# gudovskiy/contextflow

Hardware: AMD Instinct MI355X
Metric: samples/s fwd+logdet (log p(x) (B,M)), CIFAR-10C conv flow (higher is better)
Workload: dtype f32

## Files before the change

contextflow_amd/csrc/cf_step.hip:

```cpp
#include "cf_step_common.h"
#include <cstdlib>

namespace {

struct StepArgs {
    const float* x;
    float* z;
    float* ldj;
    const float* ws;
    int B;
    int64_t xbs;
    bool sq;
    hipStream_t s;
    float* dbg = nullptr;
    const float* sb = nullptr;
    StepTape tp = kNoTape;
};

constexpr int kPrepBatch = 16;
struct StepPackBatch {
    const float *Wm[kPrepBatch], *t[kPrepBatch], *logs[kPrepBatch], *w1[kPrepBatch], *b1[kPrepBatch], *w2[kPrepBatch], *b2[kPrepBatch],
        *w3[kPrepBatch], *b3[kPrepBatch];
    float* ws[kPrepBatch];
    int pieces;
// ... 166 lines not shown
            }
        }
    }
}

template <class G, bool SQ, int CTX = 0, bool DUMP = false, bool DBG = false>
__global__ __launch_bounds__(256, G::MINW) void k_flow_step(const float* __restrict__ x, float* __restrict__ z,
                                                   float* __restrict__ ldj_acc, const float* __restrict__ ws, int B,
                                                   int64_t xbs, float* __restrict__ dbg_arg, int flags,
                                                   const float* __restrict__ sb, StepTape tp) {
    float* const dbg = DBG ? dbg_arg : nullptr;
    constexpr int C = G::C, HW = G::HW, W = G::W, H = G::H, PIX = G::PIX, HALF = G::HALF, HID = G::HID;
    constexpr int PTW = G::PTW, RT03 = G::RT03, RT1 = G::RT1;
    constexpr int WPX = 32 * PTW;
    constexpr int XI = C * PTW / 8;
    extern __shared__ __align__(16) float lds[];
    float* Y0 = lds;
    float* H1 = lds + HALF * PIX;

    const int tid = threadIdx.x, lane = tid & 63, wave = tid >> 6, li = lane & 31, lk = lane >> 5;
    const int ntiles = (B + G::SPW - 1) / G::SPW;
    const int64_t dbg_cols = (int64_t)ntiles * PIX;
    (void)flags;

    int pix[PTW], pin[PTW];
#pragma unroll
    for (int q = 0; q < PTW; ++q) {
        pix[q] = (wave * PTW + q) * 32 + li;
        pin[q] = pix[q] % HW;
    }

    float4 xr[XI];
    const int tile = blockIdx.x;
    x_load<G, SQ>(xr, x, xbs, tile, B, wave, lane);
    {
        const float* __restrict__ wsl = ws;
        const int b0 = tile * G::SPW;
        int smp[PTW];
        bool live[PTW];
#pragma unroll
        for (int q = 0; q < PTW; ++q) { smp[q] = b0 + pix[q] / HW; live[q] = smp[q] < B; }

        x_to_lds<G, SQ>(xr, H1, wave, lane);
        cf_wave_sync();

        f32x16 acc0[RT03][PTW];
#pragma unroll
        for (int rt = 0; rt < RT03; ++rt)
#pragma unroll
            for (int q = 0; q < PTW; ++q) acc0[rt][q] = bias_tile(wsl + G::OFF_B0 + rt * 32, lk);
        dense_phase<G, G::KS0, G::NG0, RT03>(acc0, ws_rsrc(wsl, G::WS_FLOATS), G::OFF_A0, H1, pix, lane);
        float y1[PTW][HALF <= 16 ? 8 : 16];
#pragma unroll
        for (int q = 0; q < PTW; ++q)
#pragma unroll
            for (int r = 0; r < (HALF <= 16 ? 8 : 16); ++r) {
                const int idx = tile_row(r, lk);
                if (idx < HALF) Y0[idx * PIX + pix[q]] = acc0[0][q][r];
                y1[q][r] = (HALF <= 16) ? acc0[0][q][r + 8] : acc0[RT03 - 1][q][r];
            }
        cf_wave_sync();
        z_store<G>(z, Y0, b0, 0, B, wave, lane);
        if constexpr (DUMP) rows_store_t<G, HALF, HALF>(tp.y0, Y0, b0, B, wave, lane);
        if (dbg) {
            __syncthreads();
            for (int e = tid; e < HALF * PIX; e += 256) dbg[(int64_t)(e / PIX) * dbg_cols + (int64_t)tile * PIX + (e % PIX)] = Y0[e];
            __syncthreads();
        }

        f32x16 acc3[RT03][PTW];
        if constexpr (CTX == 0) {
            conditioner_net<G, 0, DUMP>(acc3, lds, wsl, pix, pin, lane, tid, dbg, dbg_cols, tile, nullptr, nullptr, tp, B);
        } else {
            int soff[PTW];
#pragma unroll
            for (int q = 0; q < PTW; ++q) soff[q] = min(smp[q], B - 1) * (CTX == 1 ? C : HID);
            conditioner_net<G, CTX, DUMP>(acc3, lds, wsl, pix, pin, lane, tid, dbg, dbg_cols, tile, sb, soff, tp, B);
        }

        float lsum[PTW];
#pragma unroll
        for (int q = 0; q < PTW; ++q) {
            lsum[q] = 0.f;
#pragma unroll
            for (int r = 0; r < (HALF <= 16 ? 8 : 16); ++r) {
                const int idx = tile_row(r, lk);
                if (idx < HALF) {
                    const float tt = acc3[0][q][r];
                    const float raw = (HALF <= 16) ? acc3[0][q][r + 8] : acc3[RT03 - 1][q][r];
                    const float ls = cf_log_scale(raw);
                    Y0[idx * PIX + pix[q]] = fmaf(y1[q][r], __expf(ls), tt);
                    lsum[q] += ls;
                    if constexpr (DUMP) {
                        if (live[q]) {
                            const int64_t o = ((int64_t)smp[q] * HALF + idx) * HW + pin[q];
                            tp.ls[o] = ls;
                            tp.y1[o] = y1[q][r];
                        }
                    }
                    if (dbg) {
                        float* d = dbg + (int64_t)(C + 2 * HID) * dbg_cols + (int64_t)tile * PIX + pix[q];
                        d[(int64_t)idx * dbg_cols] = tt;
                        d[(int64_t)(HALF + idx) * dbg_cols] = raw;
                    }
                }
            }
        }
        cf_wave_sync();
        z_store<G>(z, Y0, b0, HALF, B, wave, lane);
        cf_wave_sync();

        constexpr int SEG = HW < 32 ? HW : 32;
        float v[PTW];
#pragma unroll
        for (int q = 0; q < PTW; ++q) {
            v[q] = lsum[q];
#pragma unroll
            for (int o = 1; o < SEG; o <<= 1) v[q] += __shfl_xor(v[q], o, 64);
            v[q] += __shfl_xor(v[q], 32, 64);
        }
        if constexpr (HW <= 32 * PTW) {
            constexpr int TPS = HW >= 32 ? HW / 32 : 1;
#pragma unroll
            for (int q = 0; q < PTW; q += TPS) {
                float sum = v[q];
#pragma unroll
                for (int i = 1; i < TPS; ++i) sum += v[q + i];
                if (lk == 0 && (li % SEG) == 0 && live[q]) ldj_acc[smp[q]] += wsl[0] + sum;
            }
        } else {
            constexpr int TPS = HW / 32;
#pragma unroll
            for (int q = 0; q < PTW; ++q)
                if (lane == 0) Y0[wave * WPX + q] = v[q];
            __syncthreads();
            if (tid < G::SPW && b0 + tid < B) {
                float sum = 0.f;
#pragma unroll
                for (int i = 0; i < TPS; ++i) {
                    const int t = tid * TPS + i;
                    sum += Y0[(t / PTW) * WPX + (t % PTW)];
                }
                ldj_acc[b0 + tid] += wsl[0] + sum;
            }
            __syncthreads();
        }
    }
}

typedef float f32x4 __attribute__((ext_vector_type(4)));

#ifndef CF_G16W_MINW
#define CF_G16W_MINW 4
#endif
#ifdef CF_ABL_NOCONF
#define CF_ROWIDX(r, lg) ((r) * PIX + ((lg) * 16 & 63))
#else
#define CF_ROWIDX(r, lg) (((r) + (lg)) * PIX)
#endif
template <class G, bool SQ, bool DBG = false, bool DUMP = false, int CTX = 0>
__device__ __forceinline__ void flow_step_small_body(const float* x, float* z, float* __restrict__ ldj_acc, const float* __restrict__ ws,
                                                     int B, int64_t xbs, float* __restrict__ dbg, StepTape tp,
                                                     const float* __restrict__ sb = nullptr) {
    static_assert(G::SMALL, "16x16 images, one sample per workgroup, C <= 16");
    static_assert(CTX == 0 || !G::HID16, "the per-sample bias is wired into the 32-row conditioner phases (C = 16)");
    constexpr int C = G::C, W = 16, H = 16, PIX = 256, HALF = G::HALF, HID = G::HID, PTW = G::PTW;
    constexpr int XI = C * PTW / 8;
    extern __shared__ __align__(16) float lds[];
    float* Y0 = lds;
    float* H1 = lds + HALF * PIX;
    const int tid = threadIdx.x, lane = tid & 63, wave = tid >> 6, l15 = lane & 15, lg = lane >> 4;
    const int tile = blockIdx.x;
    const int colb = wave * 64 + l15;

    float4 xr[XI];
    x_load<G, SQ>(xr, x, xbs, tile, B, wave, lane);
    const ws_rsrc_t rs = ws_rsrc(ws, G::WS_FLOATS);
    x_to_lds<G, SQ>(xr, H1, wave, lane);
    if constexpr (G::LDS_W > 0) {
        float* WL = lds + (HALF + HID) * PIX;
#pragma unroll
        for (int i = 0; i < G::LDS_W / 1024; ++i)
            *reinterpret_cast<float4*>(WL + (i * 256 + tid) * 4) = ws_frag(rs, tid, G::OFF_AW + i * 1024);
    }
    cf_wave_sync();

    f32x4 acc0[4];
    {
        const float4 b = *reinterpret_cast<const float4*>(ws + G::OFF_SB0 + 4 * lg);
#pragma unroll
        for (int ct = 0; ct < 4; ++ct) { acc0[ct][0] = b.x; acc0[ct][1] = b.y; acc0[ct][2] = b.z; acc0[ct][3] = b.w; }
#pragma unroll
        for (int g = 0; g < G::SG0; ++g) {
            const float4 a = ws_frag(rs, lane, G::OFF_SA0 + g * 256);
#pragma unroll
            for (int e = 0; e < 4; ++e)
                if (4 * (4 * g + e) < C) {
#pragma unroll
                    for (int ct = 0; ct < 4; ++ct)
                        acc0[ct] = __builtin_amdgcn_mfma_f32_16x16x4f32(f4e(a, e), H1[CF_ROWIDX(4 * (4 * g + e), lg) + colb + 16 * ct],
                                                                        acc0[ct], 0, 0, 0);
                }
        }
    }
#pragma unroll
    for (int ct = 0; ct < 4; ++ct)
#pragma unroll
        for (int j = 0; j < 2; ++j)
            if (2 * lg + j < HALF) Y0[(2 * lg + j) * PIX + colb + 16 * ct] = acc0[ct][j];
    cf_wave_sync();
    z_store<G>(z, Y0, tile, 0, B, wave, lane);
    if constexpr (DUMP) rows_store_t<G, HALF, HALF>(tp.y0, Y0, tile, B, wave, lane);
    const int64_t dbg_cols = (int64_t)B * PIX;
    auto dump = [&](const float* plane, int rows, int row0) {
        __syncthreads();
        for (int e = tid; e < rows * PIX; e += 256) dbg[(int64_t)(row0 + e / PIX) * dbg_cols + (int64_t)tile * PIX + (e % PIX)] = plane[e];
        __syncthreads();
    };
    if constexpr (DBG) dump(Y0, HALF, 0);
    auto plane_mask_store = [&](unsigned* __restrict__ m) {
        const int li = lane & 31, lk = lane >> 5;
#pragma unroll
        for (int q = 0; q < PTW; ++q) {
            unsigned b = 0;
#pragma unroll
            for (int r = 0; r < 8; ++r) b |= (H1[tile_row(r, lk) * PIX + (wave * PTW + q) * 32 + li] > 0.f ? 1u : 0u) << r;
            m[((int64_t)tile * G::NPT + wave * PTW + q) * 64 + lane] = b;
        }
    };
    (void)plane_mask_store;

    if constexpr (G::DBF) {
        static_assert(!DUMP && !DBG && CTX != 2, "evaluation form only");
        direct_bf16_phases<G>(lds, ws, rs, lane, wave);
    } else if constexpr (!G::HID16) {
        const int li = lane & 31;
        int pix[PTW], pin[PTW];
#pragma unroll
        for (int q = 0; q < PTW; ++q) { pix[q] = (wave * PTW + q) * 32 + li; pin[q] = pix[q]; }
        f32x16 unused[G::RT03][PTW];
        int soff[PTW];
#pragma unroll
        for (int q = 0; q < PTW; ++q) soff[q] = tile * HID;
        conditioner_net<G, CTX == 2 ? 2 : 0, DUMP, 2>(unused, lds, ws, pix, pin, lane, tid, DBG ? dbg : nullptr, dbg_cols, tile,
// ... 43 lines not shown
#pragma unroll
            for (int d = 0; d < 3; ++d) {
                int xx = l15 + d - 1;
                xx = xx < 0 ? -xx : (xx >= W ? 2 * (W - 1) - xx : xx);
                xo[d] = HALF * PIX + lg * PIX + xx;
            }
#pragma unroll
            for (int tap = 0; tap < 9; ++tap) {
                const float4 a = ws_frag(rs, lane, G::OFF_SA2 + tap * 256);
#pragma unroll
                for (int ct = 0; ct < 4; ++ct) {
                    int yy = wave * 4 + ct + tap / 3 - 1;
                    yy = yy < 0 ? -yy : (yy >= H ? 2 * (H - 1) - yy : yy);
                    const int src = xo[tap % 3] + yy * W;
#pragma unroll
                    for (int e = 0; e < 4; ++e)
                        a2[ct] = __builtin_amdgcn_mfma_f32_16x16x4f32(f4e(a, e), lds[src + 4 * e * PIX], a2[ct], 0, 0, 0);
                }
            }
        }
        __syncthreads();
#pragma unroll
        for (int ct = 0; ct < 4; ++ct)
#pragma unroll
            for (int r = 0; r < 4; ++r) H1[(4 * lg + r) * PIX + colb + 16 * ct] = cf_relu(a2[ct][r]);
        if constexpr (DUMP) { rows_store_t<G, HID, HID>(tp.h2, H1, tile, B, wave, lane); plane_mask_store(tp.m2); }
        if constexpr (DBG) dump(H1, HID, C + HID);
        }
    }
    cf_wave_sync();

    f32x4 acc3[4];
    {
        const float4 b = *reinterpret_cast<const float4*>(ws + G::OFF_SB3 + 4 * lg);
#pragma unroll
        for (int ct = 0; ct < 4; ++ct) { acc3[ct][0] = b.x; acc3[ct][1] = b.y; acc3[ct][2] = b.z; acc3[ct][3] = b.w; }
#pragma unroll
        for (int g = 0; g < G::SG3; ++g) {
            const float4 a = ws_frag(rs, lane, G::OFF_SA3 + g * 256);
#pragma unroll
            for (int e = 0; e < 4; ++e)
                if (4 * (4 * g + e) < HID) {
#pragma unroll
                    for (int ct = 0; ct < 4; ++ct)
                        acc3[ct] = __builtin_amdgcn_mfma_f32_16x16x4f32(f4e(a, e), H1[CF_ROWIDX(4 * (4 * g + e), lg) + colb + 16 * ct],
                                                                        acc3[ct], 0, 0, 0);
                }
        }
    }
    if constexpr (CTX == 1) {
#pragma unroll
        for (int r = 0; r < 4; ++r) {
            const int ch = chan_of_row16<G>(4 * lg + r);
            const float add = ch >= 0 ? sb[(int64_t)tile * C + ch] : 0.f;
#pragma unroll
            for (int ct = 0; ct < 4; ++ct) acc3[ct][r] += add;
        }
    }
    float lsum = 0.f;
#pragma unroll
    for (int ct = 0; ct < 4; ++ct)
#pragma unroll
        for (int j = 0; j < 2; ++j)
            if (2 * lg + j < HALF) {
                const float ls = cf_log_scale(acc3[ct][j + 2]);
                Y0[(2 * lg + j) * PIX + colb + 16 * ct] = fmaf(acc0[ct][j + 2], __expf(ls), acc3[ct][j]);
                lsum += ls;
                if constexpr (DUMP) {
                    const int64_t o = ((int64_t)tile * HALF + 2 * lg + j) * PIX + colb + 16 * ct;
                    tp.ls[o] = ls;
                    tp.y1[o] = acc0[ct][j + 2];
                }
                if constexpr (DBG) {
                    float* d = dbg + (int64_t)(C + 2 * HID) * dbg_cols + (int64_t)tile * PIX + colb + 16 * ct;
                    d[(int64_t)(2 * lg + j) * dbg_cols] = acc3[ct][j];
                    d[(int64_t)(HALF + 2 * lg + j) * dbg_cols] = acc3[ct][j + 2];
                }
            }
    cf_wave_sync();
    z_store<G>(z, Y0, tile, HALF, B, wave, lane);
    cf_wave_sync();
    lsum = cf_wave_sum(lsum);
    if (lane == 0) Y0[wave * 64] = lsum;
    __syncthreads();
    if (tid == 0 && tile < B) ldj_acc[tile] += ws[0] + ((Y0[0] + Y0[64]) + (Y0[128] + Y0[192]));
}
#ifndef CF_G16WB_MINW
#define CF_G16WB_MINW 3
#endif
#ifndef CF_G16DB_MINW
#define CF_G16DB_MINW 3
#endif
template <class G, bool SQ, bool DBG = false, bool DUMP = false, int CTX = 0>
__global__ __launch_bounds__(256, G::DBF ? CF_G16DB_MINW : G::BF16S ? CF_G16WB_MINW : (G::WINO && DUMP) ? 3 : (G::WINO && G::C == 16) ? CF_G16W_MINW : G::MINW) void k_flow_step_small(const float* __restrict__ x, float* __restrict__ z,
                                                                  float* __restrict__ ldj_acc, const float* __restrict__ ws,
                                                                  int B, int64_t xbs, float* __restrict__ dbg, StepTape tp,
                                                                  const float* __restrict__ sb = nullptr) {
    flow_step_small_body<G, SQ, DBG, DUMP, CTX>(x, z, ldj_acc, ws, B, xbs, dbg, tp, sb);
}
constexpr int kChain = 4;
struct WsChain { const float* ws[kChain]; };
template <class G, bool SQ>
__global__ __launch_bounds__(256, (G::WINO && G::C == 16) ? CF_G16W_MINW : G::MINW) void k_flow_step_small_chain(const float* x, float* z, float* __restrict__ ldj_acc,
                                                                                   const WsChain wc, int nsteps, int B, int64_t xbs) {
    flow_step_small_body<G, SQ>(x, z, ldj_acc, wc.ws[0], B, xbs, nullptr, kNoTape);
    for (int st = 1; st < nsteps; ++st) {
        __syncthreads();
        flow_step_small_body<G, false>(z, z, ldj_acc, wc.ws[st], B, (int64_t)G::C * G::HW, nullptr, kNoTape);
    }
}
template <class G>
int launch_step_small_chain(const StepArgs& a, const WsChain& wc, int n) {
    const auto k = a.sq ? k_flow_step_small_chain<G, true> : k_flow_step_small_chain<G, false>;
    k<<<dim3(a.B), dim3(256), (size_t)G::LDS_FLOATS * sizeof(float), a.s>>>(a.x, a.z, a.ldj, wc, n, a.B, a.xbs);
    return 0;
}

template <class G, bool DBG = false, bool DUMP = false, int CTX = 0>
int launch_step_small(const StepArgs& a) {
    auto k = k_flow_step_small<G, false, DBG, DUMP, CTX>;
    if constexpr (CTX == 0) { if (a.sq) k = k_flow_step_small<G, true, DBG, DUMP, CTX>; }
    k<<<dim3(a.B), dim3(256), (size_t)G::LDS_FLOATS * sizeof(float), a.s>>>(a.x, a.z, a.ldj, a.ws, a.B, a.xbs, a.dbg, a.tp, a.sb);
    return 0;
}

#ifdef CF_RS_TICKS
#define RS_TICK_INIT long long tacc_[12]; for (int k_ = 0; k_ < 12; ++k_) tacc_[k_] = 0; long long tprev_ = __builtin_readcyclecounter();
#define RS_TICK(k) { const long long tn_ = __builtin_readcyclecounter(); tacc_[k] += tn_ - tprev_; tprev_ = tn_; }
#define RS_TICK_DUMP if (blockIdx.x == 0 && lane == 0) for (int k_ = 0; k_ < 12; ++k_) z[wave * 16 + k_] = (float)tacc_[k_];
#else
#define RS_TICK_INIT
#define RS_TICK(k)
#define RS_TICK_DUMP
#endif
template <class G, int NPT, bool SQ, bool DUMP = false, int KS = 2>
__device__ __forceinline__ void flow_step_rs_body(const float* x, float* z, float* __restrict__ ldj_acc, const float* __restrict__ ws, int B,
                                                  int64_t xbs, StepTape tp = kNoTape) {
    constexpr int C = G::C, HW = G::HW, W = G::W, H = G::H, HALF = G::HALF, HID = G::HID, HP = G::HP;
    constexpr int PIXR = 32 * NPT, SPWR = PIXR / HW, RT1 = G::RT1, RT03 = G::RT03;
    static_assert(RT1 * NPT == 4 && RT03 * NPT == 2 && HP == HALF && PIXR % HW == 0, "row-split geometry");
    __shared__ __align__(16) float lds[(2 * C + HID + 2 * C) * PIXR];
    float* XP = lds;
    float* Y = XP + C * PIXR;
    float* H1 = Y + C * PIXR;
    float* T = H1 + HID * PIXR;
    static_assert(KS == 2, "eight waves: the only form that is instantiated and tested");
    constexpr int NTH = 256 * KS;
    const int tid = threadIdx.x, lane = tid & 63, wave = tid >> 6, li = lane & 31, lk = lane >> 5;
    const int w4 = wave & 3, kh2 = wave >> 2;
    const int b0 = blockIdx.x * SPWR;
    const ws_rsrc_t rs = ws_rsrc(ws, G::WS_FLOATS);
    RS_TICK_INIT
// ... 411 lines not shown
        __syncthreads();
        flow_step_rs16_body<G, false>(z, z, ldj_acc, wc.ws[st], B, (int64_t)G::C * G::HW);
    }
}
template <class G>
int launch_step_rs16_chain(const StepArgs& a, const WsChain& wc, int n) {
    const auto k = a.sq ? k_flow_step_rs16_chain<G, true> : k_flow_step_rs16_chain<G, false>;
    k<<<dim3(a.B), dim3(256), 0, a.s>>>(a.x, a.z, a.ldj, wc, n, a.B, a.xbs);
    return 0;
}
template <class G, bool DUMP = false>
int launch_step_rs16(const StepArgs& a) {
    const auto k = a.sq ? k_flow_step_rs16<G, true, DUMP> : k_flow_step_rs16<G, false, DUMP>;
    k<<<dim3(a.B), dim3(256), 0, a.s>>>(a.x, a.z, a.ldj, a.ws, a.B, a.xbs, a.tp);
    return 0;
}

extern "C" int cf_slogdet_inverse_batch(int n, const float* const* Wm, int C, float* const* logabsdet, float* const* inv, cf_stream_t stream);

template <class G>
int launch_prepare(const StepPackBatch& pb, int n, float* const* winv, hipStream_t s) {
    float* lad[kPrepBatch];
    for (int i = 0; i < n; ++i) lad[i] = pb.ws[i] + 1;
    int rc = cf_slogdet_inverse_batch(n, pb.Wm, G::C, lad, winv, (cf_stream_t)s);
    if (rc) return rc;
    int blocks = (G::WS_FLOATS + 255) / 256;
    if (blocks > 512) blocks = 512;
    k_step_pack<G><<<dim3(blocks, n), dim3(256), 0, s>>>(pb);
    return 0;
}

template <class G, bool SQ, int CTX, bool DUMP, bool DBG>
int launch_step_sq(const StepArgs& a) {
    constexpr size_t lds_bytes = (size_t)G::LDS_FLOATS * sizeof(float);
    if (lds_bytes > 64 * 1024) {
        static std::atomic<uint64_t> raised{0};
        if (int rc_ = cf_raise_dynamic_lds((const void*)k_flow_step<G, SQ, CTX, DUMP, DBG>, 160 * 1024, raised, __func__)) return rc_;
    }
    const int grid = (a.B + G::SPW - 1) / G::SPW;
    k_flow_step<G, SQ, CTX, DUMP, DBG><<<dim3(grid), dim3(256), lds_bytes, a.s>>>(a.x, a.z, a.ldj, a.ws, a.B, a.xbs, a.dbg, 0, a.sb, a.tp);
    return 0;
}
template <class G, int CTX = 0, bool DUMP = false, bool DBG = false>
int launch_step(const StepArgs& a) {
    if constexpr (CTX == 0) { if (a.sq) return launch_step_sq<G, true, CTX, DUMP, DBG>(a); }
    return launch_step_sq<G, false, CTX, DUMP, DBG>(a);
}

template <class G> struct GeoInv {
    static constexpr int RTI = (G::C + 31) / 32;
    static constexpr int OFF_WINV = 0;
    static constexpr int OFF_BI = ((G::C * G::C + 3) / 4) * 4;
    static constexpr int OFF_AI = OFF_BI + RTI * 32;
    static constexpr int WS_FLOATS = OFF_AI + G::NG0 * RTI * 256;
};

template <class G>
__global__ __launch_bounds__(256) void k_step_pack_inv(const float* __restrict__ t, const float* __restrict__ logs,
                                                       float* __restrict__ wsi) {
    using I = GeoInv<G>;
    const int gtid = blockIdx.x * 256 + threadIdx.x, gsz = gridDim.x * 256;
    const float* Winv = wsi + I::OFF_WINV;
    for (int c = gtid; c < I::RTI * 32; c += gsz) {
        float s = 0.f;
        if (c < G::C)
            for (int k = 0; k < G::C; ++k) s = fmaf(Winv[c * G::C + k], t[k], s);
// ... 559 lines not shown
```

contextflow_amd/csrc/cf_step_common.h:

```cpp
#pragma once
#include <type_traits>
#include "cf_common.h"
#include <math.h>

namespace {


typedef float f32x16 __attribute__((ext_vector_type(16)));

constexpr int kWaves = 4;

template <int C_, int H_, int W_, int SPW_, int PIPE_ = 1, int ABL_ = 0, int PATCH_ = 0>
struct Geo {
    static constexpr int C = C_, H = H_, W = W_, SPW = SPW_, PIPE = PIPE_, ABL = ABL_, PATCH = PATCH_;
    static constexpr int HW = H * W;
    static constexpr int PIX = SPW * HW;
    static constexpr int HALF = C / 2;
    static constexpr int HID = 2 * C;
    static constexpr int NPT = PIX / 32;
    static constexpr int PTW = NPT / kWaves;
    static constexpr int HP = HALF <= 16 ? 16 : 32;
    static constexpr int R03 = 2 * HP;
    static constexpr int RT03 = R03 / 32;
    static constexpr int RT1 = (HID + 31) / 32;
// ... 42 lines not shown
    static constexpr int LDS_W = (CF_WINO_LDSW && PIPE_ == 3 && HID == 16 && H == 16 && W == 16 && SPW == 1) ? 16 * HID * HID : 0;
    static constexpr int DBF_FLOATS = 3 * PIX * HID / 2;
    static constexpr int LDS_FLOATS = (DBF && DBF_FLOATS > (HALF + HID) * RS) ? DBF_FLOATS : (HALF + HID) * RS + LDS_W;
    static constexpr int MINW = (160 * 1024) / (LDS_FLOATS * 4) >= 4 ? 4 : ((160 * 1024) / (LDS_FLOATS * 4) >= 2 ? 2 : 1);
    static_assert(PIX % 128 == 0 && PTW >= 1, "workgroup must own a multiple of 128 pixels");
    static_assert(!W24 || (H == 4 && W == 4 && SPW == 8) || (H == 8 && W == 8 && SPW == 4),
                  "F(2x4, 3x3): 4x4 images, 8 samples = one column tile of 16 output tiles; 8x8 images, 4 samples = two column tiles");
    static_assert(HID % 8 == 0 && C % 4 == 0, "channel counts must fill whole k-steps");
    static_assert((HW & (HW - 1)) == 0 && (W & (W - 1)) == 0, "power-of-two images");
};

template <class G> __host__ __device__ constexpr int chan_of_row(int p) {
    return ((p % G::HP) < G::HALF) ? (p / G::HP) * G::HALF + (p % G::HP) : -1;
}

template <class G> __host__ __device__ constexpr int chan_of_row16(int p) {
    return (2 * (p >> 2) + (p & 1) < G::HALF) ? ((p & 2) ? G::HALF : 0) + 2 * (p >> 2) + (p & 1) : -1;
}

__device__ __forceinline__ f32x16 bias_tile(const float* __restrict__ bias32, int lk) {
    f32x16 a;
#pragma unroll
    for (int q = 0; q < 4; ++q) {
        const float4 v = *reinterpret_cast<const float4*>(bias32 + 8 * q + 4 * lk);
        a[4 * q + 0] = v.x; a[4 * q + 1] = v.y; a[4 * q + 2] = v.z; a[4 * q + 3] = v.w;
    }
    return a;
}
__device__ __forceinline__ int tile_row(int r, int lk) { return (r & 3) + 8 * (r >> 2) + 4 * lk; }
__device__ __forceinline__ float cf_relu(float x) { return __int_as_float(max(__float_as_int(x), 0)); }
__device__ __forceinline__ float cf_log_scale(float raw) { return fmaf(-4.0f, __builtin_amdgcn_rcpf(__expf(raw) + 1.0f), 2.0f); }
__device__ __forceinline__ float f4e(const float4& v, int e) { return e == 0 ? v.x : e == 1 ? v.y : e == 2 ? v.z : v.w; }

template <int RT, int PTW>
struct GroupOps {
    float4 a[RT];
    float b[4][PTW];
};

template <int RT, int PTW>
__device__ __forceinline__ void group_mma(f32x16 (&acc)[RT][PTW], const GroupOps<RT, PTW>& o, int nsteps) {
#pragma unroll
    for (int e = 0; e < 4; ++e) {
        if (e < nsteps) {
#pragma unroll
            for (int q = 0; q < PTW; ++q)
#pragma unroll
                for (int rt = 0; rt < RT; ++rt)
                    acc[rt][q] = __builtin_amdgcn_mfma_f32_32x32x2f32(f4e(o.a[rt], e), o.b[e][q], acc[rt][q], 0, 0, 0);
        }
    }
}

typedef __amdgpu_buffer_rsrc_t ws_rsrc_t;
__device__ __forceinline__ ws_rsrc_t ws_rsrc(const float* ws, int floats) {
    return __builtin_amdgcn_make_buffer_rsrc(const_cast<float*>(ws), 0, floats * 4, 0x00020000);
}
__device__ __forceinline__ float4 ws_frag(ws_rsrc_t rs, int lane, int foff) {
    typedef int i32x4_t __attribute__((ext_vector_type(4)));
    const i32x4_t v = __builtin_amdgcn_raw_buffer_load_b128(rs, lane * 16, foff * 4, 0);
    return make_float4(__int_as_float(v.x), __int_as_float(v.y), __int_as_float(v.z), __int_as_float(v.w));
}

template <class G, int KS, int NG, int RT, class FRAG>
__device__ __forceinline__ void dense_phase_impl(f32x16 (&acc)[RT][G::PTW], FRAG frag,
                                                 const float* __restrict__ plane, const int (&pix)[G::PTW], int lane) {
    const int lk = lane >> 5;
    cf_wave_sync();
    GroupOps<RT, G::PTW> ops[2];
    auto load = [&](int g, GroupOps<RT, G::PTW>& o) {
#pragma unroll
        for (int rt = 0; rt < RT; ++rt) o.a[rt] = frag(g * RT + rt);
#pragma unroll
        for (int e = 0; e < 4; ++e)
#pragma unroll
            for (int q = 0; q < G::PTW; ++q)
                o.b[e][q] = (4 * g + e < KS) ? plane[(2 * (4 * g + e) + lk) * G::RS + pix[q]] : 0.f;
    };
    load(0, ops[0]);
#pragma unroll
    for (int g = 0; g < NG; ++g) {
        if (g + 1 < NG) load(g + 1, ops[(g + 1) & 1]);
        __builtin_amdgcn_sched_barrier(0);
        group_mma<RT, G::PTW>(acc, ops[g & 1], KS - 4 * g);
    }
}
template <class G, int KS, int NG, int RT>
__device__ __forceinline__ void dense_phase(f32x16 (&acc)[RT][G::PTW], const float4* __restrict__ frags,
                                            const float* __restrict__ plane, const int (&pix)[G::PTW], int lane) {
    dense_phase_impl<G, KS, NG, RT>(acc, [&](int i) { return frags[i * 64 + lane]; }, plane, pix, lane);
}
template <class G, int KS, int NG, int RT>
__device__ __forceinline__ void dense_phase(f32x16 (&acc)[RT][G::PTW], ws_rsrc_t rs, int foff,
// ... 99 lines not shown
    const uint64_t p = reinterpret_cast<uint64_t>(base);
    return cf_i32x4{(int)(uint32_t)p, (int)((uint32_t)(p >> 32) & 0xffffu), bytes, 0x00020000};
}
__device__ __forceinline__ void tile_store_b128(const cf_i32x4 rs, int voff, int soff, const float4 v) {
    typedef float f32x4s __attribute__((ext_vector_type(4)));
    const f32x4s d = {v.x, v.y, v.z, v.w};
#if CF_STREAM_NT
    asm volatile("buffer_store_dwordx4 %0, %1, %2, %3 offen nt\n\ts_nop 1" : : "v"(d), "v"(voff), "s"(rs), "s"(soff) : "memory");
#else
    asm volatile("buffer_store_dwordx4 %0, %1, %2, %3 offen\n\ts_nop 1" : : "v"(d), "v"(voff), "s"(rs), "s"(soff) : "memory");
#endif
}

template <class G, int NROWS, int CT>
__device__ __forceinline__ void rows_store_t(float* __restrict__ dst, const float* __restrict__ plane, int tb0, int B,
                                             int wave, int lane) {
    constexpr int WPX = 32 * G::PTW, HW = G::HW, PIX = G::RS, RPI = 256 / WPX;
    const cf_i32x4 rs = tile_rsrc_words(dst + (int64_t)tb0 * CT * HW, min(B - tb0, G::SPW) * CT * HW * 4);
    const int idx0 = lane / (WPX / 4), col = wave * WPX + 4 * (lane % (WPX / 4));
    const int voff = ((col / HW) * CT * HW + idx0 * HW + col % HW) * 4;
    cf_wave_sync();
#ifdef CF_ABL_NOSTORE
    if (tb0 >= 0) return;
#endif
#pragma unroll
    for (int i = 0; i < (NROWS + RPI - 1) / RPI; ++i) {
        if (NROWS % RPI == 0 || idx0 + i * RPI < NROWS) {
            const float4 v = *reinterpret_cast<const float4*>(&plane[(idx0 + i * RPI) * PIX + col]);
            tile_store_b128(rs, voff, i * RPI * HW * 4, v);
        }
    }
    cf_wave_sync();
}
template <class G>
__device__ __forceinline__ void rows_store_unsq(float* __restrict__ dst, const float* __restrict__ plane, int tb0, int B,
                                                int wave, int lane) {
    constexpr int WPX = 32 * G::PTW, HW = G::HW, W = G::W, PIX = G::RS, C = G::C, Q4 = WPX / 4;
    static_assert(C % 4 == 0 && W % 4 == 0, "channel quadruples, 4 pixels of one image row");
    cf_wave_sync();
    for (int it = lane; it < (C / 2) * Q4; it += 64) {
        const int j = it / Q4, col = wave * WPX + 4 * (it - j * Q4);
        const int smp = tb0 + col / HW, p = col % HW, yy = p / W, xx = p - yy * W;
        if (smp < B) {
            const float4 a = *reinterpret_cast<const float4*>(&plane[(2 * j) * PIX + col]);
            const float4 b = *reinterpret_cast<const float4*>(&plane[(2 * j + 1) * PIX + col]);
            float* d = dst + (int64_t)smp * C * HW + (j >> 1) * 4 * HW + (2 * yy + (j & 1)) * 2 * W + 2 * xx;
            *reinterpret_cast<float4*>(d) = make_float4(a.x, b.x, a.y, b.y);
            *reinterpret_cast<float4*>(d + 4) = make_float4(a.z, b.z, a.w, b.w);
        }
    }
    cf_wave_sync();
}
template <class G, int NROWS, int CT>
__device__ __forceinline__ void rows_load_t(const float* __restrict__ src, float* __restrict__ plane, int tb0, int B,
                                            int wave, int lane) {
    typedef int i32x4_t __attribute__((ext_vector_type(4)));
    constexpr int WPX = 32 * G::PTW, HW = G::HW, PIX = G::RS, RPI = 256 / WPX;
    const ws_rsrc_t rs = tile_rsrc<G, CT>(src, tb0, B);
    const int idx0 = lane / (WPX / 4), col = wave * WPX + 4 * (lane % (WPX / 4));
    const int voff = ((col / HW) * CT * HW + idx0 * HW + col % HW) * 4;
    cf_wave_sync();
#pragma unroll
    for (int i = 0; i < (NROWS + RPI - 1) / RPI; ++i) {
        if (NROWS % RPI == 0 || idx0 + i * RPI < NROWS) {
            const i32x4_t v = __builtin_amdgcn_raw_buffer_load_b128(rs, voff, i * RPI * HW * 4, 0);
            *reinterpret_cast<float4*>(&plane[(idx0 + i * RPI) * PIX + col]) =
// ... 53 lines not shown
__device__ __forceinline__ void winograd_phase2(float* __restrict__ lds, const float* __restrict__ wsl, ws_rsrc_t rs, int lane,
                                                     int wave) {
    constexpr int W = G::W, H = G::H, HW = G::HW, PIX = G::PIX, HALF = G::HALF, HID = G::HID, RT16 = G::RT16, KG4 = G::KG4;
    constexpr int RSPLIT = G::PTW == 1 ? 2 : 1, NT = G::PTW * RSPLIT / 2, NCW = 4 / RSPLIT, RTW = RT16 / RSPLIT;
    static_assert((G::PTW == 1 || G::PTW % 2 == 0) && HID % 16 == 0 && RT16 % RSPLIT == 0, "column tiles of 16 output tiles");
    const int cw = RSPLIT == 1 ? wave : wave % NCW;
    const int rt0 = RSPLIT == 1 ? 0 : __builtin_amdgcn_readfirstlane((wave / NCW) * RTW);
    typedef float f32x2w __attribute__((ext_vector_type(2)));
    float* H1 = lds + HALF * PIX;
    const int l15 = lane & 15, lg = lane >> 4;
    constexpr int TPS = HW / 4;
    int smp[NT], ty[NT], tx[NT], rpart[NT][4], cpart[NT][4];
#pragma unroll
    for (int ct = 0; ct < NT; ++ct) {
        const int tg = (cw * NT + ct) * 16 + l15, ti = tg % TPS;
        smp[ct] = tg / TPS; ty[ct] = ti / (W / 2); tx[ct] = ti % (W / 2);
#pragma unroll
        for (int a = 0; a < 4; ++a) {
            int yy = 2 * ty[ct] - 1 + a, xx = 2 * tx[ct] - 1 + a;
            yy = yy < 0 ? -yy : (yy >= H ? 2 * (H - 1) - yy : yy);
            xx = xx < 0 ? -xx : (xx >= W ? 2 * (W - 1) - xx : xx);
            rpart[ct][a] = 4 * (HALF * PIX + lg * PIX + wino_pix<G>(smp[ct] * HW, yy, 0));
            cpart[ct][a] = 4 * ((((xx ^ lg) & 1) * (W / 2)) + (xx >> 1));
        }
    }
    f32x4w Y[NT][2][2][RTW];
#pragma unroll
    for (int ct = 0; ct < NT; ++ct)
#pragma unroll
        for (int i = 0; i < 2; ++i)
#pragma unroll
            for (int j = 0; j < 2; ++j)
#pragma unroll
                for (int rt = 0; rt < RTW; ++rt) Y[ct][i][j][rt] = f32x4w{0.f, 0.f, 0.f, 0.f};
    struct WFrag { float4 a[RTW]; };
    struct WPatch { f32x2w d[NT][2][4]; };
    constexpr int KGC = KG4 < 4 ? KG4 : 4, NCH = KG4 / KGC, NGX = 4 * KGC;
    static_assert(NGX % 2 == 0, "static ping-pong");
    constexpr int B1[4] = {0, 1, 1, 1}, B2[4] = {2, 2, 2, 3};
    constexpr float S1[4] = {1.f, 1.f, -1.f, 1.f}, S2[4] = {-1.f, 1.f, 1.f, -1.f};
    constexpr float AT[2][4] = {{1.f, 1.f, 1.f, 0.f}, {0.f, 1.f, -1.f, -1.f}};
#ifndef CF_WINO_VF_MAXRT
#define CF_WINO_VF_MAXRT 4
#endif
    constexpr bool VF = RT16 <= CF_WINO_VF_MAXRT && NCH == 1 && RSPLIT == 1;
    if constexpr (VF) {
        const float* base = lds;
        constexpr int frc = G::OFF_AW;
        auto rows_of = [&](int xi, int (&r1)[NT], int (&r2)[NT]) {
#pragma unroll
            for (int ct = 0; ct < NT; ++ct) {
                r1[ct] = xi == 0 ? rpart[ct][0] : (xi == 2 ? rpart[ct][2] : rpart[ct][1]);
                r2[ct] = xi == 2 ? rpart[ct][1] : (xi == 3 ? rpart[ct][3] : rpart[ct][2]);
            }
        };
        struct WRaw { f32x2w d[NT][2][2][2]; };
        WFrag fa[2];
        WRaw raw[2];
        auto load = [&](int xi, const int (&r1)[NT], const int (&r2)[NT], int g, WFrag& fo, WRaw& o) {
            const int nu = g / KGC, kk = g % KGC;
#ifdef CF_ABL_FIXEDW
            const int fr = frc + (0 * xi * nu * kk) * 256;
#else
            const int fr = frc + ((xi * 4 + nu) * RT16 * KG4 + kk) * 256;
#endif
            if constexpr (G::LDS_W > 0) {
#pragma unroll
// ... 255 lines not shown
                        const float k0 = c0 * AT[j][nu], k1 = c1 * AT[j][nu];
#pragma unroll
                        for (int ct = 0; ct < NT; ++ct)
#pragma unroll
                            for (int rt = 0; rt < RTW; ++rt) {
                                if constexpr (decltype(has0)::value) Y[ct][0][j][rt] += k0 * M[ct][rt];
                                if constexpr (decltype(has1)::value) Y[ct][1][j][rt] += k1 * M[ct][rt];
                            }
                    }
                __builtin_amdgcn_sched_barrier(0);
            }
#pragma unroll
            for (int ct = 0; ct < NT; ++ct) { r1[ct] = r1n[ct]; r2[ct] = r2n[ct]; }
        };
        if constexpr (CF_WINO_PEEL == 2) {
            xi_body(0, std::true_type{}, std::false_type{});
            xi_body(1, std::true_type{}, std::true_type{});
            xi_body(2, std::true_type{}, std::true_type{});
            xi_body(3, std::false_type{}, std::true_type{});
        } else if constexpr (CF_WINO_PEEL) {
            xi_body(0, std::true_type{}, std::false_type{});
#pragma unroll 1
            for (int xi = 1; xi < 3; ++xi) xi_body(xi, std::true_type{}, std::true_type{});
            xi_body(3, std::false_type{}, std::true_type{});
        } else {
#pragma unroll 1
            for (int xi = 0; xi < 4; ++xi) xi_body(xi, std::true_type{}, std::true_type{});
        }
    }
    }
    __syncthreads();
#pragma unroll
    for (int rt = 0; rt < RTW; ++rt) {
        const float4 b = *reinterpret_cast<const float4*>(wsl + G::OFF_B2 + (rt0 + rt) * 16 + 4 * lg);
#pragma unroll
        for (int ct = 0; ct < NT; ++ct)
#pragma unroll
            for (int i = 0; i < 2; ++i) {
                float* dst = H1 + ((rt0 + rt) * 16 + 4 * lg) * PIX + smp[ct] * HW + (2 * ty[ct] + i) * W + 2 * tx[ct];
                const float bb[4] = {b.x, b.y, b.z, b.w};
#pragma unroll
                for (int r = 0; r < 4; ++r)
                    *reinterpret_cast<float2*>(dst + r * PIX) =
                        make_float2(cf_relu(Y[ct][i][0][rt][r] + bb[r]), cf_relu(Y[ct][i][1][rt][r] + bb[r]));
            }
    }
    if constexpr (RSPLIT > 1) __syncthreads();
    else cf_wave_sync();
}

template <class G> __device__ __forceinline__ int w24_row(int s, int y, int kq) {
    return 128 * (s >> 1) + 32 * ((y ^ (kq >> 1)) & 1) + 8 * (y >> 1) + 4 * (s & 1);
}
template <class G> __device__ __forceinline__ int w24_col(int x, int kq) {
    return 64 * ((x >> 1) & 1) + 2 * (((x >> 2) ^ (x >> 1)) & 1) + ((x ^ kq) & 1);
}
template <class G> __device__ __forceinline__ int w24_pix(int s, int y, int x, int kq) {
    if constexpr (G::H == 4) return 8 * (4 * y + ((x + y + kq) & 3)) + s;
    else return w24_row<G>(s, y, kq) + w24_col<G>(x, kq);
}

template <class G>
__device__ __forceinline__ void winograd24_phase2(float* __restrict__ lds, const float* __restrict__ wsl, ws_rsrc_t rs, int lane,
                                                  int wave) {
    constexpr int W = G::W, H = G::H, HW = G::HW, PIX = G::PIX, HALF = G::HALF, RT16 = G::RT16, KG4 = G::KG4;
    constexpr int NCT = PIX / 128;
    constexpr int RSP = kWaves / NCT;
    static_assert(G::W24 && (NCT == 1 || NCT == 2) && RT16 % RSP == 0 && W % 4 == 0, "F(2x4, 3x3) geometry");
    constexpr int RTW = RT16 / RSP;
    constexpr int TPS = HW / 8, TXN = W / 4;
    constexpr int NS = 6 * KG4;
    constexpr int NU[6] = {0, 5, 1, 2, 3, 4};
    typedef float f32x2w __attribute__((ext_vector_type(2)));
    const int rt0 = __builtin_amdgcn_readfirstlane((NCT == 1 ? wave : wave / NCT) * RTW);
    float* H1 = lds + HALF * PIX;
    const int l15 = lane & 15, lg = lane >> 4;
    const int tg = (wave % NCT) * 16 + l15;
    const int smp = H == 4 ? l15 >> 1 : tg / TPS, ty = H == 4 ? l15 & 1 : (tg % TPS) / TXN, tx = H == 4 ? 0 : tg % TXN;
    int yrow[4], xcol[6];
#pragma unroll
    for (int a = 0; a < 4; ++a) {
        const int yy = 2 * ty - 1 + a;
        yrow[a] = yy < 0 ? -yy : (yy >= H ? 2 * (H - 1) - yy : yy);
    }
#pragma unroll
    for (int c = 0; c < 6; ++c) {
        const int xx = 4 * tx - 1 + c;
        xcol[c] = xx < 0 ? -xx : (xx >= W ? 2 * (W - 1) - xx : xx);
    }
    int cpart[6];
    if constexpr (H != 4) {
#pragma unroll
        for (int c = 0; c < 6; ++c) cpart[c] = 4 * (HALF * PIX + lg * PIX + w24_col<G>(xcol[c], lg));
    }
    f32x4w Y[2][4][RTW];
#pragma unroll
    for (int i = 0; i < 2; ++i)
#pragma unroll
        for (int j = 0; j < 4; ++j)
#pragma unroll
            for (int rt = 0; rt < RTW; ++rt) Y[i][j][rt] = f32x4w{0.f, 0.f, 0.f, 0.f};
    auto addrs = [&](int xi, int (&o)[2][6]) {
#pragma unroll
        for (int h = 0; h < 2; ++h) {
            const int yy = h == 0 ? (xi == 0 ? yrow[0] : (xi == 2 ? yrow[2] : yrow[1]))
                                  : (xi == 2 ? yrow[1] : (xi == 3 ? yrow[3] : yrow[2]));
#pragma unroll
            for (int c = 0; c < 6; ++c) {
                if constexpr (H == 4) {
                    const int xx = c == 0 ? 1 : (c == 5 ? 2 : c - 1);
                    o[h][c] = 4 * (HALF * PIX + lg * PIX + w24_pix<G>(smp, yy, xx, lg & 1));
                } else {
                    o[h][c] = 4 * w24_row<G>(smp, yy, lg) + cpart[c];
                }
            }
        }
    };
    struct Raw { f32x2w d[2][6][2]; };
    struct WFrag { float4 a[RTW]; };
    auto load_raw = [&](const int (&o)[2][6], int kk, Raw& r) {
#pragma unroll
        for (int h = 0; h < 2; ++h)
#pragma unroll
            for (int c = 0; c < 6; ++c)
#pragma unroll
                for (int e2 = 0; e2 < 2; ++e2) {
                    const char* q0 = reinterpret_cast<const char*>(lds) + (16 * kk + 8 * e2) * PIX * 4;
                    const char* q1 = q0 + 4 * PIX * 4;
                    r.d[h][c][e2] = f32x2w{*reinterpret_cast<const float*>(q0 + o[h][c]), *reinterpret_cast<const float*>(q1 + o[h][c])};
                }
    };
    auto load_w = [&](int xi, int s, WFrag& f) {
        const int kk = s / 6, nu = NU[s % 6];
        const int fr = G::OFF_AW24 + (((xi * 6 + nu) * RT16 + rt0) * KG4 + kk) * 256;
// ... 42 lines not shown
                    else if (nu == 1) v[e2] = (a4 - 0.25f * a2) + (a3 - 0.25f * a1);
                    else if (nu == 2) v[e2] = (a4 - 0.25f * a2) - (a3 - 0.25f * a1);
                    else if (nu == 3) v[e2] = (a4 - a2) + 0.5f * (a3 - a1);
                    else if (nu == 4) v[e2] = (a4 - a2) - 0.5f * (a3 - a1);
                    else v[e2] = 0.25f * a1 + (a5 - 1.25f * a3);
                }
                const WFrag& f = wf[s & 1];
#pragma unroll
                for (int e = 0; e < 4; ++e)
#pragma unroll
                    for (int rt = 0; rt < RTW; ++rt)
                        M[nu][rt] = __builtin_amdgcn_mfma_f32_16x16x4f32(f4e(f.a[rt], e), v[e >> 1][e & 1], M[nu][rt], 0, 0, 0);
                __builtin_amdgcn_sched_barrier(0);
            }
        }
#pragma unroll
        for (int rt = 0; rt < RTW; ++rt) {
            const f32x4w s12 = M[1][rt] + M[2][rt], d12 = M[1][rt] - M[2][rt], s34 = M[3][rt] + M[4][rt], d34 = M[3][rt] - M[4][rt];
            const f32x4w Z[4] = {M[0][rt] + s12 + s34, d12 + 0.5f * d34, s12 + 0.25f * s34, d12 + 0.125f * d34 + M[5][rt]};
#pragma unroll
            for (int j = 0; j < 4; ++j) {
                if constexpr (decltype(has0)::value) Y[0][j][rt] += c0 * Z[j];
                if constexpr (decltype(has1)::value) Y[1][j][rt] += c1 * Z[j];
            }
        }
    };
    xi_body(0, std::true_type{}, std::false_type{});
#pragma unroll 1
    for (int xi = 1; xi < 3; ++xi) xi_body(xi, std::true_type{}, std::true_type{});
    xi_body(3, std::false_type{}, std::true_type{});
    __syncthreads();
#pragma unroll
    for (int rt = 0; rt < RTW; ++rt) {
        const float4 b = *reinterpret_cast<const float4*>(wsl + G::OFF_B2 + (rt0 + rt) * 16 + 4 * lg);
        const float bb[4] = {b.x, b.y, b.z, b.w};
#pragma unroll
        for (int i = 0; i < 2; ++i)
#pragma unroll
            for (int r = 0; r < 4; ++r) {
                float* dst = H1 + ((rt0 + rt) * 16 + 4 * lg + r) * PIX + smp * HW + (2 * ty + i) * W + (H == 4 ? 0 : 4 * tx);
                *reinterpret_cast<float4*>(dst) = make_float4(cf_relu(Y[i][0][rt][r] + bb[r]), cf_relu(Y[i][1][rt][r] + bb[r]),
                                                              cf_relu(Y[i][2][rt][r] + bb[r]), cf_relu(Y[i][3][rt][r] + bb[r]));
            }
    }
    __syncthreads();
}

template <class G>
__device__ __forceinline__ void direct_bf16_phases(float* __restrict__ lds, const float* __restrict__ wsl, ws_rsrc_t rs, int lane, int wave) {
    static_assert(G::DBF && G::H == 16 && G::W == 16 && G::SPW == 1 && G::HID == 32 && G::PTW == 2, "the 16x16 level at C = 16");
    constexpr int PIX = G::PIX, HALF = G::HALF, HID = G::HID, PTW = G::PTW, RT16 = G::RT16;
    constexpr int PLANE = PIX * HID * 2;
    typedef __bf16 bf16x8w __attribute__((ext_vector_type(8)));
    float* Y0 = lds;
    float* H1 = lds + HALF * PIX;
    char* const ldsb = reinterpret_cast<char*>(lds);
    const int li = lane & 31, lk = lane >> 5, l15 = lane & 15, lg = lane >> 4;
    int pix[PTW];
#pragma unroll
    for (int q = 0; q < PTW; ++q) pix[q] = (wave * PTW + q) * 32 + li;
    f32x16 acc1[1][PTW];
#pragma unroll
    for (int q = 0; q < PTW; ++q) acc1[0][q] = bias_tile(wsl + G::OFF_B1, lk);
    dense_phase<G, G::KS1, G::NG1, 1>(acc1, rs, G::OFF_A1, Y0, pix, lane);
    float4 wp[2][RT16][3];
    auto wp_load = [&](float4 (&dst)[RT16][3], int tap) {
#pragma unroll
        for (int rt = 0; rt < RT16; ++rt)
#pragma unroll
            for (int pz = 0; pz < 3; ++pz) dst[rt][pz] = ws_frag(rs, lane, G::OFF_ADB + ((tap * RT16 + rt) * 3 + pz) * 256);
    };
    wp_load(wp[0], 0);
    __syncthreads();
#pragma unroll
    for (int q = 0; q < PTW; ++q) {
// ... 377 lines not shown
```

Before: 3.698 million.

## Use DPP lane reductions, seed Winograd accumulators with bias, add buffer I/O path

Wave and segment reductions of the log-scale sum now use DPP and permlane swap instructions instead of ds_bpermute shuffles. The conv-phase accumulators start from the bias, which drops a bias add from the epilogue. Bias loads in the small-image path go through buffer loads. An optional buffer-resource load and store path for the x and z tiles is added with a stride check, but it is disabled by default, so the x and z I/O stays on the old path. Each change removes a few instructions and moves some work to other units, at the risk of slightly different rounding from the earlier bias addition.

```diff
diff --git a/contextflow_amd/csrc/cf_step.hip b/contextflow_amd/csrc/cf_step.hip
--- a/contextflow_amd/csrc/cf_step.hip
+++ b/contextflow_amd/csrc/cf_step.hip
@@ -222,7 +222,7 @@
 
     float4 xr[XI];
     const int tile = blockIdx.x;
-    x_load<G, SQ>(xr, x, xbs, tile, B, wave, lane);
+    x_load_b<G, SQ>(xr, x, xbs, tile, B, wave, lane);
     {
         const float* __restrict__ wsl = ws;
         const int b0 = tile * G::SPW;
@@ -250,7 +250,7 @@
                 y1[q][r] = (HALF <= 16) ? acc0[0][q][r + 8] : acc0[RT03 - 1][q][r];
             }
         cf_wave_sync();
-        z_store<G>(z, Y0, b0, 0, B, wave, lane);
+        z_store_b<G>(z, Y0, b0, 0, B, wave, lane);
         if constexpr (DUMP) rows_store_t<G, HALF, HALF>(tp.y0, Y0, b0, B, wave, lane);
         if (dbg) {
             __syncthreads();
@@ -297,17 +297,19 @@
             }
         }
         cf_wave_sync();
-        z_store<G>(z, Y0, b0, HALF, B, wave, lane);
+        z_store_b<G>(z, Y0, b0, HALF, B, wave, lane);
         cf_wave_sync();
 
         constexpr int SEG = HW < 32 ? HW : 32;
         float v[PTW];
 #pragma unroll
         for (int q = 0; q < PTW; ++q) {
-            v[q] = lsum[q];
-#pragma unroll
-            for (int o = 1; o < SEG; o <<= 1) v[q] += __shfl_xor(v[q], o, 64);
-            v[q] += __shfl_xor(v[q], 32, 64);
+            v[q] = cf_xor_add<1>(lsum[q]);
+            if constexpr (SEG > 2) v[q] = cf_xor_add<2>(v[q]);
+            if constexpr (SEG > 4) v[q] = cf_xor_add<4>(v[q]);
+            if constexpr (SEG > 8) v[q] = cf_xor_add<8>(v[q]);
+            if constexpr (SEG > 16) v[q] = cf_xor_add<16>(v[q]);
+            v[q] = cf_xor_add<32>(v[q]);
         }
         if constexpr (HW <= 32 * PTW) {
             constexpr int TPS = HW >= 32 ? HW / 32 : 1;
@@ -364,7 +366,7 @@
     const int colb = wave * 64 + l15;
 
     float4 xr[XI];
-    x_load<G, SQ>(xr, x, xbs, tile, B, wave, lane);
+    x_load_b<G, SQ>(xr, x, xbs, tile, B, wave, lane);
     const ws_rsrc_t rs = ws_rsrc(ws, G::WS_FLOATS);
     x_to_lds<G, SQ>(xr, H1, wave, lane);
     if constexpr (G::LDS_W > 0) {
@@ -377,7 +379,7 @@
 
     f32x4 acc0[4];
     {
-        const float4 b = *reinterpret_cast<const float4*>(ws + G::OFF_SB0 + 4 * lg);
+        const float4 b = ws_f4(rs, 16 * lg, G::OFF_SB0);
 #pragma unroll
         for (int ct = 0; ct < 4; ++ct) { acc0[ct][0] = b.x; acc0[ct][1] = b.y; acc0[ct][2] = b.z; acc0[ct][3] = b.w; }
 #pragma unroll
@@ -399,7 +401,7 @@
         for (int j = 0; j < 2; ++j)
             if (2 * lg + j < HALF) Y0[(2 * lg + j) * PIX + colb + 16 * ct] = acc0[ct][j];
     cf_wave_sync();
-    z_store<G>(z, Y0, tile, 0, B, wave, lane);
+    z_store_b<G>(z, Y0, tile, 0, B, wave, lane);
     if constexpr (DUMP) rows_store_t<G, HALF, HALF>(tp.y0, Y0, tile, B, wave, lane);
     const int64_t dbg_cols = (int64_t)B * PIX;
     auto dump = [&](const float* plane, int rows, int row0) {
@@ -509,7 +511,7 @@
 
     f32x4 acc3[4];
     {
-        const float4 b = *reinterpret_cast<const float4*>(ws + G::OFF_SB3 + 4 * lg);
+        const float4 b = ws_f4(rs, 16 * lg, G::OFF_SB3);
 #pragma unroll
         for (int ct = 0; ct < 4; ++ct) { acc3[ct][0] = b.x; acc3[ct][1] = b.y; acc3[ct][2] = b.z; acc3[ct][3] = b.w; }
 #pragma unroll
@@ -555,9 +557,9 @@
                 }
             }
     cf_wave_sync();
-    z_store<G>(z, Y0, tile, HALF, B, wave, lane);
+    z_store_b<G>(z, Y0, tile, HALF, B, wave, lane);
     cf_wave_sync();
-    lsum = cf_wave_sum(lsum);
+    lsum = cf_wave_sum_dpp(lsum);
     if (lane == 0) Y0[wave * 64] = lsum;
     __syncthreads();
     if (tid == 0 && tile < B) ldj_acc[tile] += ws[0] + ((Y0[0] + Y0[64]) + (Y0[128] + Y0[192]));
@@ -586,8 +588,13 @@
         flow_step_small_body<G, false>(z, z, ldj_acc, wc.ws[st], B, (int64_t)G::C * G::HW, nullptr, kNoTape);
     }
 }
+static int stride_too_large(const char* fn, int64_t xbs) {
+    cf_set_error("%s: batch stride %lld: a workgroup's samples do not fit a 31-bit byte offset", fn, (long long)xbs);
+    return CF_ERR_UNSUPPORTED;
+}
 template <class G>
 int launch_step_small_chain(const StepArgs& a, const WsChain& wc, int n) {
+    if (!tile_span_fits<G>(a.xbs)) return stride_too_large(__func__, a.xbs);
     const auto k = a.sq ? k_flow_step_small_chain<G, true> : k_flow_step_small_chain<G, false>;
     k<<<dim3(a.B), dim3(256), (size_t)G::LDS_FLOATS * sizeof(float), a.s>>>(a.x, a.z, a.ldj, wc, n, a.B, a.xbs);
     return 0;
@@ -595,6 +602,7 @@
 
 template <class G, bool DBG = false, bool DUMP = false, int CTX = 0>
 int launch_step_small(const StepArgs& a) {
+    if (!tile_span_fits<G>(a.xbs)) return stride_too_large(__func__, a.xbs);
     auto k = k_flow_step_small<G, false, DBG, DUMP, CTX>;
     if constexpr (CTX == 0) { if (a.sq) k = k_flow_step_small<G, true, DBG, DUMP, CTX>; }
     k<<<dim3(a.B), dim3(256), (size_t)G::LDS_FLOATS * sizeof(float), a.s>>>(a.x, a.z, a.ldj, a.ws, a.B, a.xbs, a.dbg, a.tp, a.sb);
@@ -1072,6 +1080,7 @@
 
 template <class G, bool SQ, int CTX, bool DUMP, bool DBG>
 int launch_step_sq(const StepArgs& a) {
+    if (!tile_span_fits<G>(a.xbs)) return stride_too_large(__func__, a.xbs);
     constexpr size_t lds_bytes = (size_t)G::LDS_FLOATS * sizeof(float);
     if (lds_bytes > 64 * 1024) {
         static std::atomic<uint64_t> raised{0};
diff --git a/contextflow_amd/csrc/cf_step_common.h b/contextflow_amd/csrc/cf_step_common.h
--- a/contextflow_amd/csrc/cf_step_common.h
+++ b/contextflow_amd/csrc/cf_step_common.h
@@ -98,6 +98,39 @@
 __device__ __forceinline__ float cf_log_scale(float raw) { return fmaf(-4.0f, __builtin_amdgcn_rcpf(__expf(raw) + 1.0f), 2.0f); }
 __device__ __forceinline__ float f4e(const float4& v, int e) { return e == 0 ? v.x : e == 1 ? v.y : e == 2 ? v.z : v.w; }
 
+#ifndef CF_BIAS_FIRST
+#define CF_BIAS_FIRST 1
+#endif
+
+#ifndef CF_DPP_SUM
+#define CF_DPP_SUM 1
+#endif
+template <int O> __device__ __forceinline__ float cf_xor_add(float v) {
+    static_assert(O == 1 || O == 2 || O == 4 || O == 8 || O == 16 || O == 32, "lane distance inside a wave");
+#if CF_DPP_SUM
+    const unsigned u = __float_as_uint(v);
+    if constexpr (O == 1) return v + __uint_as_float(__builtin_amdgcn_update_dpp(0, u, 0xB1, 0xf, 0xf, true));
+    else if constexpr (O == 2) return v + __uint_as_float(__builtin_amdgcn_update_dpp(0, u, 0x4E, 0xf, 0xf, true));
+    else if constexpr (O == 4) {
+        const unsigned t = __builtin_amdgcn_update_dpp(0, u, 0x141, 0xf, 0xf, true);
+        return v + __uint_as_float(__builtin_amdgcn_update_dpp(0, t, 0x1B, 0xf, 0xf, true));
+    } else if constexpr (O == 8) return v + __uint_as_float(__builtin_amdgcn_update_dpp(0, u, 0x128, 0xf, 0xf, true));
+    else if constexpr (O == 16) {
+        const auto r = __builtin_amdgcn_permlane16_swap(u, u, false, false);
+        return __uint_as_float(r[0]) + __uint_as_float(r[1]);
+    } else {
+        const auto r = __builtin_amdgcn_permlane32_swap(u, u, false, false);
+        return __uint_as_float(r[0]) + __uint_as_float(r[1]);
+    }
+#else
+    return v + __shfl_xor(v, O, 64);
+#endif
+}
+__device__ __forceinline__ float cf_wave_sum_dpp(float v) {
+    v = cf_xor_add<32>(v); v = cf_xor_add<16>(v); v = cf_xor_add<8>(v);
+    v = cf_xor_add<4>(v); v = cf_xor_add<2>(v); return cf_xor_add<1>(v);
+}
+
 template <int RT, int PTW>
 struct GroupOps {
     float4 a[RT];
@@ -125,6 +158,12 @@
 __device__ __forceinline__ float4 ws_frag(ws_rsrc_t rs, int lane, int foff) {
     typedef int i32x4_t __attribute__((ext_vector_type(4)));
     const i32x4_t v = __builtin_amdgcn_raw_buffer_load_b128(rs, lane * 16, foff * 4, 0);
+    return make_float4(__int_as_float(v.x), __int_as_float(v.y), __int_as_float(v.z), __int_as_float(v.w));
+}
+
+__device__ __forceinline__ float4 ws_f4(ws_rsrc_t rs, int voff, int foff) {
+    typedef int i32x4_t __attribute__((ext_vector_type(4)));
+    const i32x4_t v = __builtin_amdgcn_raw_buffer_load_b128(rs, voff, foff * 4, 0);
     return make_float4(__int_as_float(v.x), __int_as_float(v.y), __int_as_float(v.z), __int_as_float(v.w));
 }
 
@@ -290,6 +329,61 @@
     }
     cf_wave_sync();
 }
+#ifndef CF_BUF_IO
+#define CF_BUF_IO 0
+#endif
+template <class G> inline bool tile_span_fits(int64_t xbs) { return !CF_BUF_IO || (int64_t)G::SPW * xbs * 4 < (1ll << 31); }
+template <class G, bool SQ>
+__device__ __forceinline__ void x_load_b(float4 (&xr)[G::C * G::PTW / 8], const float* x, int64_t xbs, int tile, int B, int wave, int lane) {
+#if !CF_BUF_IO
+    x_load<G, SQ>(xr, x, xbs, tile, B, wave, lane);
+#else
+    typedef int i32x4_t __attribute__((ext_vector_type(4)));
+    constexpr int WPX = 32 * G::PTW, HW = G::HW, W = G::W;
+    constexpr int Q = SQ ? WPX / 2 : WPX / 4;
+    constexpr int K = 64 / Q;
+    static_assert(64 % Q == 0 && (!SQ || K % 2 == 0), "an item adds a constant to every lane's offset");
+    const int tb0 = tile * G::SPW, xs = (int)xbs;
+    const ws_rsrc_t rs = __builtin_amdgcn_make_buffer_rsrc(const_cast<float*>(x + (int64_t)tb0 * xbs), 0, min(B - tb0, G::SPW) * xs * 4, 0x00020000);
+    const int r0 = lane / Q;
+    int voff;
+    if constexpr (!SQ) {
+        const int col = wave * WPX + 4 * (lane % Q);
+        voff = ((col / HW) * xs + r0 * HW + col % HW) * 4;
+    } else {
+        const int col = wave * WPX + 2 * (lane % Q), p = col % HW, yy = p / W, xx = p % W;
+        voff = ((col / HW) * xs + (r0 >> 1) * 4 * HW + (2 * yy + (r0 & 1)) * 2 * W + 2 * xx) * 4;
+    }
+#pragma unroll
+    for (int i = 0; i < G::C * G::PTW / 8; ++i) {
+        const int soff = (SQ ? i * (K / 2) * 4 * HW : i * K * HW) * 4;
+        const i32x4_t v = __builtin_amdgcn_raw_buffer_load_b128(rs, voff, soff, CF_STREAM_NT ? 2 : 0);
+        xr[i] = make_float4(__int_as_float(v.x), __int_as_float(v.y), __int_as_float(v.z), __int_as_float(v.w));
+    }
+#endif
+}
+template <class G>
+__device__ __forceinline__ void z_store_b(float* z, const float* __restrict__ plane, int tb0, int ch0, int B, int wave, int lane) {
+#if !CF_BUF_IO
+    z_store<G>(z, plane, tb0, ch0, B, wave, lane);
+#else
+    constexpr int WPX = 32 * G::PTW, HW = G::HW, PIX = G::RS, C = G::C, NROWS = G::HALF, Q = WPX / 4, RPI = 64 / Q;
+    static_assert(64 % Q == 0, "whole channel rows per item");
+    const cf_i32x4 rs = tile_rsrc_words(z + (int64_t)tb0 * C * HW, min(B - tb0, G::SPW) * C * HW * 4);
+    const int idx0 = lane / Q, col = wave * WPX + 4 * (lane % Q);
+    const int voff = ((col / HW) * C * HW + idx0 * HW + col % HW) * 4;
+    cf_wave_sync();
+#pragma unroll
+    for (int i = 0; i < (NROWS + RPI - 1) / RPI; ++i) {
+        if (NROWS % RPI == 0 || idx0 + i * RPI < NROWS) {
+            const float4 v = *reinterpret_cast<const float4*>(&plane[(idx0 + i * RPI) * PIX + col]);
+            tile_store_b128(rs, voff, (ch0 + i * RPI) * HW * 4, v);
+        }
+    }
+    cf_wave_sync();
+#endif
+}
+
 template <class G>
 __device__ __forceinline__ void rows_store_unsq(float* __restrict__ dst, const float* __restrict__ plane, int tb0, int B,
                                                 int wave, int lane) {
@@ -409,7 +503,14 @@
 #pragma unroll
             for (int j = 0; j < 2; ++j)
 #pragma unroll
-                for (int rt = 0; rt < RTW; ++rt) Y[ct][i][j][rt] = f32x4w{0.f, 0.f, 0.f, 0.f};
+                for (int rt = 0; rt < RTW; ++rt) {
+                    if constexpr (CF_BIAS_FIRST) {
+                        const float4 b = ws_f4(rs, 16 * lg, G::OFF_B2 + (rt0 + rt) * 16);
+                        Y[ct][i][j][rt] = f32x4w{b.x, b.y, b.z, b.w};
+                    } else {
+                        Y[ct][i][j][rt] = f32x4w{0.f, 0.f, 0.f, 0.f};
+                    }
+                }
     struct WFrag { float4 a[RTW]; };
     struct WPatch { f32x2w d[NT][2][4]; };
     constexpr int KGC = KG4 < 4 ? KG4 : 4, NCH = KG4 / KGC, NGX = 4 * KGC;
@@ -731,17 +832,21 @@
     __syncthreads();
 #pragma unroll
     for (int rt = 0; rt < RTW; ++rt) {
-        const float4 b = *reinterpret_cast<const float4*>(wsl + G::OFF_B2 + (rt0 + rt) * 16 + 4 * lg);
+        float bb[4] = {0.f, 0.f, 0.f, 0.f};
+        if constexpr (!CF_BIAS_FIRST) {
+            const float4 b = *reinterpret_cast<const float4*>(wsl + G::OFF_B2 + (rt0 + rt) * 16 + 4 * lg);
+            bb[0] = b.x; bb[1] = b.y; bb[2] = b.z; bb[3] = b.w;
+        }
 #pragma unroll
         for (int ct = 0; ct < NT; ++ct)
 #pragma unroll
             for (int i = 0; i < 2; ++i) {
                 float* dst = H1 + ((rt0 + rt) * 16 + 4 * lg) * PIX + smp[ct] * HW + (2 * ty[ct] + i) * W + 2 * tx[ct];
-                const float bb[4] = {b.x, b.y, b.z, b.w};
 #pragma unroll
                 for (int r = 0; r < 4; ++r)
                     *reinterpret_cast<float2*>(dst + r * PIX) =
-                        make_float2(cf_relu(Y[ct][i][0][rt][r] + bb[r]), cf_relu(Y[ct][i][1][rt][r] + bb[r]));
+                        CF_BIAS_FIRST ? make_float2(cf_relu(Y[ct][i][0][rt][r]), cf_relu(Y[ct][i][1][rt][r]))
+                                      : make_float2(cf_relu(Y[ct][i][0][rt][r] + bb[r]), cf_relu(Y[ct][i][1][rt][r] + bb[r]));
             }
     }
     if constexpr (RSPLIT > 1) __syncthreads();
@@ -798,7 +903,14 @@
 #pragma unroll
         for (int j = 0; j < 4; ++j)
 #pragma unroll
-            for (int rt = 0; rt < RTW; ++rt) Y[i][j][rt] = f32x4w{0.f, 0.f, 0.f, 0.f};
+            for (int rt = 0; rt < RTW; ++rt) {
+                if constexpr (CF_BIAS_FIRST) {
+                    const float4 b = ws_f4(rs, 16 * lg, G::OFF_B2 + (rt0 + rt) * 16);
+                    Y[i][j][rt] = f32x4w{b.x, b.y, b.z, b.w};
+                } else {
+                    Y[i][j][rt] = f32x4w{0.f, 0.f, 0.f, 0.f};
+                }
+            }
     auto addrs = [&](int xi, int (&o)[2][6]) {
 #pragma unroll
         for (int h = 0; h < 2; ++h) {
@@ -907,15 +1019,20 @@
     __syncthreads();
 #pragma unroll
     for (int rt = 0; rt < RTW; ++rt) {
-        const float4 b = *reinterpret_cast<const float4*>(wsl + G::OFF_B2 + (rt0 + rt) * 16 + 4 * lg);
-        const float bb[4] = {b.x, b.y, b.z, b.w};
+        float bb[4] = {0.f, 0.f, 0.f, 0.f};
+        if constexpr (!CF_BIAS_FIRST) {
+            const float4 b = *reinterpret_cast<const float4*>(wsl + G::OFF_B2 + (rt0 + rt) * 16 + 4 * lg);
+            bb[0] = b.x; bb[1] = b.y; bb[2] = b.z; bb[3] = b.w;
+        }
 #pragma unroll
         for (int i = 0; i < 2; ++i)
 #pragma unroll
             for (int r = 0; r < 4; ++r) {
                 float* dst = H1 + ((rt0 + rt) * 16 + 4 * lg + r) * PIX + smp * HW + (2 * ty + i) * W + (H == 4 ? 0 : 4 * tx);
-                *reinterpret_cast<float4*>(dst) = make_float4(cf_relu(Y[i][0][rt][r] + bb[r]), cf_relu(Y[i][1][rt][r] + bb[r]),
-                                                              cf_relu(Y[i][2][rt][r] + bb[r]), cf_relu(Y[i][3][rt][r] + bb[r]));
+                *reinterpret_cast<float4*>(dst) =
+                    CF_BIAS_FIRST ? make_float4(cf_relu(Y[i][0][rt][r]), cf_relu(Y[i][1][rt][r]), cf_relu(Y[i][2][rt][r]), cf_relu(Y[i][3][rt][r]))
+                                  : make_float4(cf_relu(Y[i][0][rt][r] + bb[r]), cf_relu(Y[i][1][rt][r] + bb[r]),
+                                                cf_relu(Y[i][2][rt][r] + bb[r]), cf_relu(Y[i][3][rt][r] + bb[r]));
             }
     }
     __syncthreads();
```

Result: no change. 3.726 million, median of 6 (+0.7%).
